# byronknoll/gmix

Measured on AMD Instinct MI355X. Metric: mixer bits/sec (synthetic 256-input mixer streams, forward+update), higher is better.
Workload: dtype f32; 1 GPU; configs[1]: synthetic 256-input 1-layer mixer (1 mixer, 2^16-row gate table), random logits, forward+update; n_inputs=256, mixers=1/0/0, streams_per_gpu=4096, total_bits=5486149632, parallelism=streams sharded over 1 GPU(s), no collective on the data path

## Files before the change

### gmix_amd/csrc/gmx_capi.cpp

```cpp
#include <hip/hip_runtime.h>
#include <math.h>
#include <stddef.h>
#include <stdio.h>
#include <stdlib.h>
#include <string.h>
#include <time.h>

#include <algorithm>
#include <atomic>
#include <map>
#include <new>
#include <string>
#include <vector>

#include "../../include/gmxmix.h"
#include "../../include/gmxmix_lstm_group.h"
#include "../../include/gmxmix_decoder.h"
#include "gmx_buildhash.h"
#include "gmx_internal.h"
#include "gmx_mailbox.h"
#include "gmx_batch_rows.h"
#include "gmx_ckpt.h"
#include "gmx_ckpt_stage.h"
#include "gmx_ind_ckpt.h"
// ... 284 lines not shown
  if (k->up) {
    const size_t bytes = (size_t)c->S * n * gmx_cols_row_bytes(c->cols, dir);
    int rc = up ? xfer_begin_upload(c->x, main, k->up, bytes, &st) : xfer_begin_download(c->x, main, k->down, bytes, &st);
    if (rc) return rc;
  }
  for (const GmxBatchCol& col : c->cols) {
    if (col.dir != dir || col.per_stream) continue;
    void *dst = up ? *col.dev : *col.host, *src = up ? *col.host : *col.dev;
    const GmxRowCopy r = gmx_row_copy(c->S, c->max_rows, n, col.row_bytes);
    if (r.height)
      HIPCHK(hipMemcpy2DAsync(dst, r.pitch, src, r.pitch, r.width, r.height, kind, st));
    else
      HIPCHK(hipMemcpyAsync(dst, src, r.bytes, kind, st));
  }
  for (const GmxBatchCol& col : c->cols) {
    if (col.dir != dir || !col.per_stream) continue;
    void *dst = up ? *col.dev : *col.host, *src = up ? *col.host : *col.dev;
    HIPCHK(hipMemcpyAsync(dst, src, gmx_col_host_bytes(col, c->S, c->max_rows), kind, st));
  }
  return up ? xfer_end_upload(c->x, main, st) : xfer_end_download(c->x, st);
}
static int batch_core_wait(GmxBatchCore* c) {
  if (!c || !c->bank) return GMX_ERR_INVALID;
  HIPCHK(hipSetDevice(c->bank->device));
  return xfer_wait(c->x);
}


static constexpr int kStageSlots = 4;
struct GmxCountList {
  uint64_t* dev[kStageSlots] = {};
  uint64_t* host[kStageSlots] = {};
  hipEvent_t done[kStageSlots] = {};
  bool busy[kStageSlots] = {};
  size_t cap = 0;
  unsigned seq = 0;
};
static void count_list_free(GmxCountList& c) {
  for (int k = 0; k < kStageSlots; ++k) {
    if (c.dev[k]) (void)hipFree(c.dev[k]);
    if (c.host[k]) (void)hipHostFree(c.host[k]);
    if (c.done[k]) (void)hipEventDestroy(c.done[k]);
  }
  c = GmxCountList();
}
static int count_list_stage(GmxCountList& c, const uint64_t* counts, int n, hipStream_t st, const uint64_t** dev_out) {
  const int k = (int)(c.seq++ % (unsigned)kStageSlots);
  if (c.busy[k]) {
    HIPCHK(hipEventSynchronize(c.done[k]));
    c.busy[k] = false;
  }
  if ((size_t)n > c.cap) {
    for (int j = 0; j < kStageSlots; ++j) {
      if (c.busy[j]) {
        HIPCHK(hipEventSynchronize(c.done[j]));
        c.busy[j] = false;
      }
      if (c.dev[j]) (void)hipFree(c.dev[j]);
      if (c.host[j]) (void)hipHostFree(c.host[j]);
      c.dev[j] = nullptr;
      c.host[j] = nullptr;
    }
    c.cap = 0;
    const size_t cap = (size_t)n + 64;
    for (int j = 0; j < kStageSlots; ++j) {
      HIPCHK(hipMalloc((void**)&c.dev[j], cap * sizeof(uint64_t)));
      HIPCHK(hipHostMalloc((void**)&c.host[j], cap * sizeof(uint64_t), hipHostMallocDefault));
      if (!c.done[j]) HIPCHK(hipEventCreateWithFlags(&c.done[j], hipEventDisableTiming));
    }
    c.cap = cap;
  }
  memcpy(c.host[k], counts, (size_t)n * sizeof(uint64_t));
  HIPCHK(hipMemcpyAsync(c.dev[k], c.host[k], (size_t)n * sizeof(uint64_t), hipMemcpyHostToDevice, st));
  *dev_out = c.dev[k];
  return GMX_OK;
}
static int count_list_used(GmxCountList& c, hipStream_t st) {
  const int k = (int)((c.seq - 1u) % (unsigned)kStageSlots);
  HIPCHK(hipEventRecord(c.done[k], st));
  c.busy[k] = true;
  return GMX_OK;
}

struct gmx_group {
  int device = 0;
  int S = 0;
  GmxTopoDev topo;
  GmxTopoDev* topo_dev = nullptr;
  uint8_t* banks = nullptr;
  float* latch_out = nullptr;
  hipStream_t stream = nullptr;
  hipEvent_t ev0 = nullptr, ev1 = nullptr;
  unsigned lds_bytes = 0;
  std::vector<uint64_t> steps;
  std::vector<uint8_t> fwd_done;
  struct DecaySlot {
    float* dev = nullptr;
    uint32_t* idx_dev = nullptr;
    float* host = nullptr;
    uint32_t* idx_host = nullptr;
    size_t cap = 0;
    size_t idx_cap = 0;
    hipEvent_t done = nullptr;
    hipEvent_t ready = nullptr;
    bool busy = false;
    uint64_t* st_dev = nullptr;
    uint64_t* st_host = nullptr;
    uint32_t* amb_dev = nullptr;
    uint32_t* amb_host = nullptr;
    float* patch_host = nullptr;
    size_t st_cap = 0;
  } decay[kStageSlots];
  GmxCountList counts;
  hipStream_t copy_stream = nullptr;
  hipStream_t up_stream = nullptr, down_stream = nullptr;
  unsigned run_seq = 0;
  hipEvent_t tm0 = nullptr, tm1 = nullptr;
  gmx_batch* one = nullptr;
  GmxBatchBank bb;
  std::vector<struct GmxSession*> sessions;
  std::vector<struct gmx_lockstep*> locksteps;
  bool banks_in_use_by_dead_kernel = false;
  bool use_sessions = true;
  bool mailbox_on_device = true;
  bool force_general = false;
  bool stock_exact = false;
  int stock_staged = -1;
  bool decay_on_host = false;
  bool stock_pairs = false;
  bool register_rows = false;
  int single_variant = 0;
  struct GmxCkptState* ckpt = nullptr;
};

struct gmx_batch : GmxBatchCore {
  gmx_group* g = nullptr;
  uint64_t& max_bits = max_rows;
  unsigned flags = 0;
  float* d_pred = nullptr;
  uint32_t* d_mask = nullptr;
  uint32_t* d_ctx = nullptr;
  uint8_t* d_bits = nullptr;
  float* d_p = nullptr;
  float* d_out = nullptr;
  float* d_last = nullptr;
  uint64_t* d_rng = nullptr;
  uint64_t* d_tcount = nullptr;
  float* d_pstate = nullptr;
  uint32_t* d_cstate = nullptr;
  float* h_pred = nullptr;
  uint32_t* h_mask = nullptr;
  uint32_t* h_ctx = nullptr;
  uint8_t* h_bits = nullptr;
  float* h_p = nullptr;
  float* h_out = nullptr;
  float* h_last = nullptr;
};

struct gmx_lockstep {
  gmx_group* g = nullptr;
  gmx_batch* b = nullptr;
  float* dec_host = nullptr;
  uint8_t* bits_host = nullptr;
  float* dec_dev = nullptr;
  uint32_t* idx_dev = nullptr;
  hipGraph_t g_predict = nullptr, g_learn = nullptr, g_step = nullptr;
  hipGraphExec_t x_predict = nullptr, x_learn = nullptr, x_step = nullptr;
  bool predicted = false;
  bool persistent = false, ps_running = false, ps_dead = false, ps_counted = false;
  hipStream_t ps_stream = nullptr;
  GmxLsDoor* door = nullptr;
  uint32_t* done = nullptr;
  uint32_t* blk_seen = nullptr;
// ... 125 lines not shown
      x.rs_off = x.w_off + (uint64_t)at * 4u;
      x.rs_pitch = x.stride * 4u;
    } else {
      x.rs_off = off;
      x.rs_pitch = 8u;
      off += (uint64_t)x.table_size * 8u;
      off = round_up64(off, 128);
    }
  }
  o->scal_off = off;
  off += (uint64_t)o->m * 24u;
  o->bank_bytes = round_up64(off, 256);
  uint32_t l = 0;
  o->lds_in0 = l;
  o->in0_sz = round_up((uint32_t)o->n_pad + (uint32_t)o->l0 + 4u, 4);
  l += 2 * o->in0_sz;
  o->lds_o1 = l;
  l += round_up((uint32_t)(o->l1 ? o->l1 : 1), 4);
  o->lds_skip = l;
  l += GMX_MAX_SKIP;
  o->lds_misc = l;
  l += 256;
  for (int grp = 0; grp < 2; ++grp) {
    const int lo = grp == 0 ? 0 : o->l0, hi = grp == 0 ? o->l0 : o->m;
    if (lo >= hi) continue;
    uint32_t dmax = 0;
    for (int j = lo; j < hi; ++j) dmax = std::max(dmax, o->mx[j].stride);
    const uint32_t D = dmax + 4;
    const uint32_t S = round_up((uint32_t)(hi - lo) * D, 64);
    for (int j = lo; j < hi; ++j) {
      o->mx[j].lds_off = l + (uint32_t)(j - lo) * D;
      o->mx[j].pitch = S;
    }
    l += 2 * S;
  }
  o->lds_total = l;
  if ((uint64_t)o->lds_total * 4u > 160u * 1024u) return GMX_ERR_INVALID;
  return GMX_OK;
}

static void batch_free(gmx_batch* b);
static int batch_alloc(gmx_batch** out, gmx_group* g, int S, uint64_t max_bits, unsigned flags);
static int batch_note_device_use(gmx_batch* b);

extern "C" int gmx_group_create(gmx_group** out, const gmx_topology* topo, int n_streams, int device) {
  if (!out || n_streams < 1) return GMX_ERR_INVALID;
  *out = nullptr;
  GmxTopoDev td;
  int rc = build_topology(topo, &td);
  if (rc) return rc;
  int ndev = 0;
  if (hipGetDeviceCount(&ndev) != hipSuccess || ndev <= 0) {
    (void)hipGetLastError();
    return GMX_ERR_NO_DEVICE;
  }
  if (device < 0 || device >= ndev) return GMX_ERR_INVALID;
  HIPCHK(hipSetDevice(device));
  gmx_group* g = new (std::nothrow) gmx_group();
  if (!g) return GMX_ERR_NOMEM;
  g->device = device;
  batch_bank_init(g->bb, g, device, &g->stream, &g->up_stream, &g->down_stream);
  g->S = n_streams;
  g->topo = td;
  g->lds_bytes = td.lds_total * 4u;
  g->steps.assign(n_streams, 0);
  g->fwd_done.assign(n_streams, 0);
#define GCHK(call)                                 \
  do {                                             \
    hipError_t e_ = (call);                        \
    if (e_ != hipSuccess) {                        \
      int r_ = hip_fail(e_, #call);                \
      gmx_group_destroy(g);                        \
      return e_ == hipErrorOutOfMemory ? GMX_ERR_NOMEM : r_; \
    }                                              \
  } while (0)
  GCHK(bank_stream_create(&g->stream, 0));
  GCHK(hipEventCreate(&g->ev0));
  GCHK(hipEventCreate(&g->ev1));
  GCHK(hipMalloc((void**)&g->topo_dev, sizeof(GmxTopoDev)));
  GCHK(hipMemcpy(g->topo_dev, &g->topo, sizeof(GmxTopoDev), hipMemcpyHostToDevice));
  GCHK(hipMalloc((void**)&g->banks, (size_t)n_streams * td.bank_bytes));
  GCHK(hipMalloc((void**)&g->latch_out, (size_t)n_streams * td.m * sizeof(float)));
  GCHK(hipMemsetAsync(g->latch_out, 0, (size_t)n_streams * td.m * sizeof(float), g->stream));
  if (g->lds_bytes > 48u * 1024u) GCHK(gmx_bank_kernel_set_lds(g->lds_bytes));
#undef GCHK
  rc = gmx_group_reset(g);
  if (rc) {
    gmx_group_destroy(g);
    return rc;
  }
  *out = g;
  return GMX_OK;
}

extern "C" void gmx_group_destroy(gmx_group* g) {
  if (!g) return;
  (void)hipSetDevice(g->device);
  sessions_free(g);
  if (g->stream) (void)hipStreamSynchronize(g->stream);
  if (g->one) {
    batch_free(g->one);
    g->one = nullptr;
  }
  for (gmx_lockstep* ls : g->locksteps) ls->g = nullptr;
  g->locksteps.clear();
  batch_bank_detach_all(g->bb);
  if (!g->banks_in_use_by_dead_kernel) {
    if (g->banks) (void)hipFree(g->banks);
    if (g->latch_out) (void)hipFree(g->latch_out);
    if (g->topo_dev) (void)hipFree(g->topo_dev);
  }
  for (auto& d : g->decay) {
    if (d.st_dev) (void)hipFree(d.st_dev);
    if (d.st_host) (void)hipHostFree(d.st_host);
    if (d.amb_dev) (void)hipFree(d.amb_dev);
    if (d.amb_host) (void)hipHostFree(d.amb_host);
    if (d.patch_host) (void)hipHostFree(d.patch_host);
    if (d.dev) (void)hipFree(d.dev);
    if (d.idx_dev) (void)hipFree(d.idx_dev);
    if (d.host) (void)hipHostFree(d.host);
    if (d.idx_host) (void)hipHostFree(d.idx_host);
    if (d.done) (void)hipEventDestroy(d.done);
    if (d.ready) (void)hipEventDestroy(d.ready);
  }
  count_list_free(g->counts);
  ckpt_free(g);
  if (g->copy_stream) (void)hipStreamDestroy(g->copy_stream);
  if (g->up_stream) {
    (void)hipStreamSynchronize(g->up_stream);
    (void)hipStreamDestroy(g->up_stream);
  }
  if (g->down_stream) {
    (void)hipStreamSynchronize(g->down_stream);
    (void)hipStreamDestroy(g->down_stream);
  }
  if (g->tm0) (void)hipEventDestroy(g->tm0);
  if (g->tm1) (void)hipEventDestroy(g->tm1);
  if (g->ev0) (void)hipEventDestroy(g->ev0);
  if (g->ev1) (void)hipEventDestroy(g->ev1);
  if (g->stream) (void)hipStreamDestroy(g->stream);
  delete g;
}

extern "C" int gmx_group_n_streams(const gmx_group* g) { return g ? g->S : GMX_ERR_INVALID; }
extern "C" int gmx_group_n_mixers(const gmx_group* g) { return g ? g->topo.m : GMX_ERR_INVALID; }
extern "C" int gmx_group_n_inputs(const gmx_group* g) { return g ? g->topo.n : GMX_ERR_INVALID; }
extern "C" uint64_t gmx_group_bank_bytes(const gmx_group* g) { return g ? g->topo.bank_bytes : 0; }

extern "C" int gmx_group_reset(gmx_group* g) {
  if (!g) return GMX_ERR_INVALID;
  HIPCHK(hipSetDevice(g->device));
  int rc = sessions_close(g, false);
  if (rc) return rc;
  HIPCHK(hipMemsetAsync(g->banks, 0, (size_t)g->S * g->topo.bank_bytes, g->stream));
  HIPCHK(gmx_launch_init_scal(g->banks, g->topo.bank_bytes, g->topo.scal_off, g->topo.m, g->S,
                              g->stream));
  HIPCHK(hipStreamSynchronize(g->stream));
  std::fill(g->steps.begin(), g->steps.end(), 0);
  std::fill(g->fwd_done.begin(), g->fwd_done.end(), 0);
  for (gmx_lockstep* ls : g->locksteps) ls->predicted = false;
  return GMX_OK;
}

extern "C" int gmx_group_sync(gmx_group* g) {
  if (!g) return GMX_ERR_INVALID;
  HIPCHK(hipSetDevice(g->device));
  int rc = sessions_close(g, true);
  if (rc) return rc;
  HIPCHK(hipStreamSynchronize(g->stream));
  return GMX_OK;
}

extern "C" int gmx_group_timer_start(gmx_group* g) {
  if (!g) return GMX_ERR_INVALID;
  HIPCHK(hipSetDevice(g->device));
  if (!g->tm0) {
    HIPCHK(hipEventCreate(&g->tm0));
    HIPCHK(hipEventCreate(&g->tm1));
  }
  HIPCHK(hipEventRecord(g->tm0, g->stream));
  return GMX_OK;
}

extern "C" int gmx_group_timer_stop(gmx_group* g, float* ms) {
  if (!g || !ms || !g->tm0) return GMX_ERR_INVALID;
  HIPCHK(hipSetDevice(g->device));
  HIPCHK(hipEventRecord(g->tm1, g->stream));
  HIPCHK(hipEventSynchronize(g->tm1));
  HIPCHK(hipEventElapsedTime(ms, g->tm0, g->tm1));
  return GMX_OK;
}

// ... 99 lines not shown
      }
      if (!e.done) {
        HIPCHK(hipEventCreateWithFlags(&e.done, hipEventDisableTiming));
        HIPCHK(hipEventCreateWithFlags(&e.ready, hipEventDisableTiming));
      }
    }
  }
  if (!g->copy_stream) HIPCHK(sibling_stream_create(&g->copy_stream, g->stream));
  bool on_device = false;
  if (learn && uniq.size() > 1 && uniq.size() * T >= kDecayDeviceMin && uniq.size() * T < (1ull << 32) &&
      !g->decay_on_host) {
    const int rcd = decay_table_on_device(g, d, uniq, T);
    if (rcd != GMX_OK && rcd != GMX_ERR_STATE) return rcd;
    on_device = rcd == GMX_OK;
  }
  if (!on_device) {
    for (auto& kv : uniq) {
      float* tab = d.host + (size_t)kv.second * T;
      if (learn)
        for (uint64_t t = 0; t < T; ++t) tab[t] = decay_base(kv.first + t);
      else
        for (uint64_t t = 0; t < T; ++t) tab[t] = 0.f;
    }
    HIPCHK(hipMemcpyAsync(d.dev, d.host, uniq.size() * T * sizeof(float), hipMemcpyHostToDevice, g->copy_stream));
  }
  memcpy(d.idx_host, idx.data(), ns * sizeof(uint32_t));
  HIPCHK(hipMemcpyAsync(d.idx_dev, d.idx_host, ns * sizeof(uint32_t), hipMemcpyHostToDevice, g->copy_stream));
  HIPCHK(hipEventRecord(d.ready, g->copy_stream));
  HIPCHK(hipStreamWaitEvent(g->stream, d.ready, 0));
  return GMX_OK;
}

static bool topo_register_rows_eligible(const GmxTopoDev& t) {
  return t.has_final && t.l0 >= 1 && t.l0 <= 24 && t.l1 >= 1 && t.l1 <= 8 && t.m == t.l0 + t.l1 + 1 &&
         t.n_skip == 1 && gmx_pair_kernel_half(t.n) != 0;
}

enum GmxKernelKind : int { GMX_K_SINGLE, GMX_K_WIDE, GMX_K_STOCK, GMX_K_BANK, GMX_K_PAIR };
static GmxKernelKind kernel_for(const gmx_group* g, unsigned mode) {
  if (g->register_rows && (mode & GMX_MODE_PREDICT) && !(mode & GMX_MODE_LATCH) && !g->force_general &&
      topo_register_rows_eligible(g->topo))
    return GMX_K_PAIR;
  const bool single = g->topo.m == 1 && g->topo.n <= 256 && (mode & GMX_MODE_PREDICT) &&
                      !(mode & GMX_MODE_LATCH) && !g->force_general;
  const bool stock = g->topo.n == 90 && g->topo.l0 == 24 && g->topo.l1 == 8 && g->topo.n_skip == 1 &&
                     g->topo.has_final && g->topo.mx[23].stride == 128 && !g->force_general;
  const bool wide = g->topo.l0 == 24 && g->topo.l1 == 8 && g->topo.n_skip == 1 && g->topo.has_final &&
                    ((g->topo.n == 256 && g->topo.mx[23].stride == 288) ||
                     (g->topo.n == 90 && g->topo.mx[23].stride == 128 && g->stock_pairs && !g->stock_exact)) &&
                    (mode & GMX_MODE_PREDICT) && !(mode & GMX_MODE_LATCH) && !g->force_general;
  return single ? GMX_K_SINGLE : wide ? GMX_K_WIDE : stock ? GMX_K_STOCK : GMX_K_BANK;
}

static int launch_run(gmx_group* g, gmx_batch* b, int s0, int rec0, int ns, uint64_t T,
                      unsigned mode, float* kernel_ms, const uint64_t* n_list = nullptr) {
  if (T == 0) return GMX_OK;
  for (gmx_lockstep* ls : g->locksteps) ls->predicted = false;
  gmx_group::DecaySlot* dec = nullptr;
  int rc = prepare_decay(g, s0, ns, T, (mode & GMX_MODE_LEARN) ? 1 : 0, &dec);
  if (rc) return rc;
  GmxRunArgs a;
  memset(&a, 0, sizeof a);
  a.banks = g->banks;
  a.pred = b->d_pred;
  a.mask = (b->flags & GMX_BATCH_MASK) ? b->d_mask : nullptr;
  a.ctx = b->d_ctx;
  a.bits = b->d_bits;
  a.decay = dec->dev;
  a.decay_idx = dec->idx_dev;
  a.p_out = b->d_p;
  a.out_all = (b->flags & GMX_BATCH_OUTPUTS) ? b->d_out : nullptr;
  a.out_last = (b->flags & GMX_BATCH_LAST_OUTPUTS) ? b->d_last : nullptr;
  a.latch_out = g->latch_out;
  a.rec_stride = b->max_bits;
  a.T = T;
  if (n_list) {
    int rcl = count_list_stage(g->counts, n_list, ns, g->stream, &a.T_list);
    if (rcl) return rcl;
  }
  a.mode = mode | (g->stock_exact ? GMX_MODE_EXACT : 0u);
  a.stream_base = s0;
  a.rec_base = rec0;
  a.n_streams = ns;
  {
    int rcx = xfer_before_run(b->x, g->stream);
    if (rcx) return rcx;
  }
  if (kernel_ms) HIPCHK(hipEventRecord(g->ev0, g->stream));
  const GmxKernelKind kind = kernel_for(g, mode);
  const bool single = kind == GMX_K_SINGLE, wide = kind == GMX_K_WIDE, stock = kind == GMX_K_STOCK;
  if (a.out_last && (single || wide)) return GMX_ERR_INVALID;
  if (kind == GMX_K_PAIR)
    HIPCHK(gmx_launch_pair_kernel(g->topo_dev, &a, ns, a.mask != nullptr, g->topo.n, g->topo.l0, g->topo.l1, g->stream));
  else if (single)
    HIPCHK(gmx_launch_single_kernel(g->topo_dev, &a, g->topo.n, g->single_variant, g->stream));
  else if (wide)
    HIPCHK(gmx_launch_wide_kernel(g->topo_dev, &a, ns, a.mask != nullptr, g->topo.n, g->stream));
  else if (stock)
    HIPCHK(gmx_launch_stock_kernel(g->topo_dev, &a, ns, GMX_STK_LDS_BYTES(g->topo.lds_misc),
                                   a.mask != nullptr, g->stock_staged, topo_tables_pow2(g->topo), g->stream));
  else
    HIPCHK(gmx_launch_bank_kernel(g->topo_dev, &a, ns, g->lds_bytes, a.mask != nullptr, g->topo.l0,
                                  g->topo.l1, g->topo.n_skip, g->topo.has_final,
                                  g->topo.mx[g->topo.l0 - 1].stride, g->stream));
  HIPCHK(hipEventRecord(dec->done, g->stream));
  dec->busy = true;
  if (n_list) {
    int rcl = count_list_used(g->counts, g->stream);
    if (rcl) return rcl;
  }
  {
    int rcn = batch_note_device_use(b);
    if (rcn) return rcn;
  }
  if (kernel_ms) {
    HIPCHK(hipEventRecord(g->ev1, g->stream));
    HIPCHK(hipEventSynchronize(g->ev1));
    HIPCHK(hipEventElapsedTime(kernel_ms, g->ev0, g->ev1));
  }
  if (mode & GMX_MODE_LEARN)
    for (int i = 0; i < ns; ++i) g->steps[s0 + i] += n_list ? n_list[i] : T;
  return GMX_OK;
}

static void batch_free(gmx_batch* b) {
  if (!b) return;
  batch_core_free(*b);
  delete b;
}

static int batch_alloc(gmx_batch** out, gmx_group* g, int S, uint64_t max_bits, unsigned flags) {
  if (!out || !g || max_bits == 0) return GMX_ERR_INVALID;
  *out = nullptr;
  gmx_batch* b = new (std::nothrow) gmx_batch();
  if (!b) return GMX_ERR_NOMEM;
  b->back = (void**)&b->g;
  b->flags = flags;
  gmx_mixer_batch_cols(b->cols, b, g->topo.n_pad, g->topo.m, g->topo.mask_words, flags);
  int rc = batch_core_alloc(*b, &g->bb, S, max_bits, false);
  if (rc) {
    batch_free(b);
    return rc;
  }
  *out = b;
  return GMX_OK;
}

extern "C" int gmx_batch_create(gmx_batch** out, gmx_group* g, uint64_t max_bits, unsigned flags) {
  if (!g) return GMX_ERR_INVALID;
  if (flags & GMX_BATCH_LAST_OUTPUTS) {
    const GmxKernelKind kind = kernel_for(g, GMX_MODE_PREDICT | GMX_MODE_LEARN);
    if ((kind == GMX_K_SINGLE || kind == GMX_K_WIDE) && !topo_register_rows_eligible(g->topo)) return GMX_ERR_INVALID;
  }
  int rc = batch_alloc(out, g, g->S, max_bits, flags);
  if (rc) return rc;
  return xfer_streams_ready(g->stream, &g->up_stream, &g->down_stream);
}

extern "C" void gmx_batch_destroy(gmx_batch* b) { batch_free(b); }
extern "C" int gmx_batch_n_pad(const gmx_batch* b) { return (b && b->g) ? b->g->topo.n_pad : GMX_ERR_INVALID; }
extern "C" int gmx_batch_mask_words(const gmx_batch* b) { return (b && b->g) ? b->g->topo.mask_words : GMX_ERR_INVALID; }
extern "C" uint64_t gmx_batch_max_bits(const gmx_batch* b) { return b ? b->max_bits : 0; }

extern "C" float* gmx_batch_predictions(gmx_batch* b) { return b ? (float*)batch_core_host(*b, &b->h_pred) : nullptr; }
extern "C" uint32_t* gmx_batch_active_mask(gmx_batch* b) {
  return b ? (uint32_t*)batch_core_host(*b, &b->h_mask) : nullptr;
// ... 260 lines not shown
      memcpy(rs, p + 4, 8);
      if (*rs == 0) return GMX_ERR_FORMAT;
      memcpy(w + (size_t)r * x.stride, p + 12, 4 * (size_t)input_size);
      p += 12 + 4 * (size_t)input_size;
    }
  }
  if (p != end) return GMX_ERR_FORMAT;
  HIPCHK(hipSetDevice(g->device));
  int rc = sessions_close(g, true);
  if (rc) return rc;
  if (stream < (int)g->sessions.size() && g->sessions[stream]) g->sessions[stream]->fwd_live = false;
  HIPCHK(hipStreamSynchronize(g->stream));
  HIPCHK(hipMemcpy(g->banks + (size_t)stream * t.bank_bytes, img.data(), img.size(),
                   hipMemcpyHostToDevice));
  g->steps[stream] = sc[0];
  g->fwd_done[stream] = 0;
  for (gmx_lockstep* ls : g->locksteps) ls->predicted = false;
  return GMX_OK;
}

extern "C" int gmx_bank_copy(gmx_group* dst, int dst_stream, gmx_group* src, int src_stream) {
  if (!dst || !src || dst_stream < 0 || dst_stream >= dst->S || src_stream < 0 || src_stream >= src->S)
    return GMX_ERR_INVALID;
  const GmxTopoDev &a = dst->topo, &b = src->topo;
  if (a.m != b.m || a.n != b.n || a.n_skip != b.n_skip || a.bank_bytes != b.bank_bytes)
    return GMX_ERR_INVALID;
  for (int j = 0; j < a.m; ++j)
    if (a.mx[j].table_size != b.mx[j].table_size || a.mx[j].weight_size != b.mx[j].weight_size ||
        a.mx[j].layer != b.mx[j].layer)
      return GMX_ERR_INVALID;
  HIPCHK(hipSetDevice(src->device));
  int rc = sessions_close(src, true);
  if (rc) return rc;
  HIPCHK(hipStreamSynchronize(src->stream));
  HIPCHK(hipSetDevice(dst->device));
  rc = sessions_close(dst, true);
  if (rc) return rc;
  if (dst_stream < (int)dst->sessions.size() && dst->sessions[dst_stream])
    dst->sessions[dst_stream]->fwd_live = false;
  HIPCHK(hipStreamSynchronize(dst->stream));
  HIPCHK(hipMemcpy(dst->banks + (size_t)dst_stream * a.bank_bytes,
                   src->banks + (size_t)src_stream * b.bank_bytes, a.bank_bytes,
                   hipMemcpyDeviceToDevice));
  dst->steps[dst_stream] = src->steps[src_stream];
  dst->fwd_done[dst_stream] = 0;
  for (gmx_lockstep* ls : dst->locksteps) ls->predicted = false;
  return GMX_OK;
}

#include "gmx_ckpt.inc"

extern "C" int gmx_bank_memory_usage(gmx_group* g, int stream, int mixer, uint64_t* bytes) {
  if (!g || stream < 0 || stream >= g->S || mixer < 0 || mixer >= g->topo.m || !bytes)
    return GMX_ERR_INVALID;
  HIPCHK(hipSetDevice(g->device));
  int rc = sessions_close(g, true);
  if (rc) return rc;
  HIPCHK(hipStreamSynchronize(g->stream));
  uint64_t sc[3];
  HIPCHK(hipMemcpy(sc, g->banks + (size_t)stream * g->topo.bank_bytes + g->topo.scal_off + 24u * mixer,
                   24, hipMemcpyDeviceToHost));
  const GmxMixerDev& x = g->topo.mx[mixer];
  *bytes = 29 + sc[2] * (uint64_t)(x.weight_size * 4 + 12) + 8ull * x.table_size;
  return GMX_OK;
}


#include "gmx_indirect.inc"
#include "gmx_ind_ckpt.inc"
#include "gmx_lstm.inc"
#include "gmx_lstm_ckpt.inc"
#include "gmx_match.inc"
#include "gmx_match_ckpt.inc"
#include "gmx_ctx.inc"
#include "gmx_ctx_ckpt.inc"
#include "gmx_chainstep.inc"
#include "gmx_coder.inc"

extern "C" int gmx_debug_single_variant(gmx_group* g, int lanes_per_stream) {
  if (!g || (lanes_per_stream != 0 && lanes_per_stream != 16 && lanes_per_stream != 32 &&
             lanes_per_stream != 64 && lanes_per_stream != 165 && lanes_per_stream != 325))
    return GMX_ERR_INVALID;
  g->single_variant = lanes_per_stream;
  return GMX_OK;
}

extern "C" int gmx_debug_stock_pairs(gmx_group* g, int on) {
  if (!g) return GMX_ERR_INVALID;
  g->stock_pairs = on != 0;
  return GMX_OK;
}

extern "C" int gmx_debug_decay_on_host(gmx_group* g, int on) {
  if (!g) return GMX_ERR_INVALID;
  g->decay_on_host = on != 0;
  return GMX_OK;
}

extern "C" int gmx_debug_decay_table(gmx_group* g, const uint64_t* steps0, int U, uint64_t T, float* out,
                                     uint32_t* n_unsettled) {
  if (!g || !steps0 || U < 1 || T < 1 || !out) return GMX_ERR_INVALID;
  HIPCHK(hipSetDevice(g->device));
  if (!g->copy_stream) HIPCHK(sibling_stream_create(&g->copy_stream, g->stream));
  gmx_group::DecaySlot tmp;
  std::map<uint64_t, uint32_t> uniq;
  std::vector<uint32_t> row(U);
  for (int u = 0; u < U; ++u) {
    auto it = uniq.find(steps0[u]);
    if (it == uniq.end()) it = uniq.emplace(steps0[u], (uint32_t)uniq.size()).first;
    row[u] = it->second;
  }
  HIPCHK(hipMalloc((void**)&tmp.dev, uniq.size() * T * sizeof(float)));
  int rc = decay_table_on_device(g, tmp, uniq, T);
  if (rc == GMX_OK) {
    if (n_unsettled) *n_unsettled = tmp.amb_host[0];
    std::vector<float> h(uniq.size() * T);
    hipError_t e = hipMemcpyAsync(h.data(), tmp.dev, h.size() * sizeof(float), hipMemcpyDeviceToHost, g->copy_stream);
    if (e == hipSuccess) e = hipStreamSynchronize(g->copy_stream);
    if (e != hipSuccess) rc = hip_fail(e, "gmx_debug_decay_table copy");
    else
      for (int u = 0; u < U; ++u) memcpy(out + (size_t)u * T, h.data() + (size_t)row[u] * T, T * sizeof(float));
  }
  void* dv[] = {tmp.dev, tmp.st_dev, tmp.amb_dev};
  for (void* p : dv)
    if (p) (void)hipFree(p);
  void* hv[] = {tmp.st_host, tmp.amb_host, tmp.patch_host};
  for (void* p : hv)
    if (p) (void)hipHostFree(p);
  return rc;
}

extern "C" int gmx_topology_register_rows_eligible(const gmx_topology* topo) {
  GmxTopoDev td;
  if (build_topology(topo, &td) != GMX_OK) return GMX_ERR_INVALID;
  return topo_register_rows_eligible(td) ? 1 : 0;
}

extern "C" int gmx_group_set_register_rows(gmx_group* g, int on) {
  if (!g || !topo_register_rows_eligible(g->topo)) return GMX_ERR_INVALID;
  g->register_rows = on != 0;
  return GMX_OK;
}

extern "C" int gmx_debug_force_general(gmx_group* g, int on) {
  if (!g) return GMX_ERR_INVALID;
  g->force_general = on != 0;
  return GMX_OK;
}

extern "C" int gmx_debug_kernel_kind(gmx_group* g, unsigned mode) {
  if (!g) return GMX_ERR_INVALID;
  const GmxKernelKind kind = kernel_for(g, mode);
  if (kind != GMX_K_BANK) return (int)kind;
  const GmxTopoDev& t = g->topo;
  return (int)kind + 4 * gmx_bank_kernel_build(t.l0, t.l1, t.n_skip, t.has_final, t.mx[t.l0 - 1].stride);
}

extern "C" int gmx_debug_stock_staged(gmx_group* g, int mode) {
  if (!g || mode < -1 || mode > 1) return GMX_ERR_INVALID;
  g->stock_staged = mode;
  return GMX_OK;
}

extern "C" int gmx_debug_stock_exact(gmx_group* g, int on) {
  if (!g) return GMX_ERR_INVALID;
  int rc = sessions_close(g, true);
// ... 511 lines not shown
```

### gmix_amd/csrc/gmx_internal.h

```cpp
#ifndef GMX_INTERNAL_H_
#define GMX_INTERNAL_H_

#include <stdint.h>

#define GMX_MAX_MIXERS 64
#define GMX_MAX_SKIP 8
#define GMX_MAX_INPUTS 2048

#define GMX_MODE_PREDICT 1u
#define GMX_MODE_LEARN 2u
#define GMX_MODE_LATCH 4u
#define GMX_MODE_EXACT 8u

struct GmxMixerDev {
  uint32_t table_size;
  uint32_t weight_size;
  uint32_t stride;
  uint32_t lds_off;
  uint32_t pitch;
  int32_t layer;
  int32_t out_index;
  float lr;
  uint64_t w_off;
  uint64_t rs_off;
  uint32_t rs_pitch;
  uint32_t rs_folded;
};

#define GMX_RS_PTR(bank, mx, row) \
  ((uint64_t*)((uint8_t*)(bank) + (mx).rs_off + (uint64_t)(row) * (mx).rs_pitch))

struct GmxTopoDev {
  int32_t n, n_pad, n_skip, m, l0, l1, has_final, mask_words;
  int32_t skip_idx[GMX_MAX_SKIP];
  uint32_t lds_in0;
  uint32_t in0_sz;
  uint32_t lds_o1;
  uint32_t lds_skip;
  uint32_t lds_misc;
  uint32_t lds_total;
  uint64_t scal_off;
  uint64_t bank_bytes;
  GmxMixerDev mx[GMX_MAX_MIXERS];
};

struct GmxRunArgs {
  uint8_t* banks;
  const float* pred;
  const uint32_t* mask;
  const uint32_t* ctx;
  const uint8_t* bits;
  const float* decay;
  const uint32_t* decay_idx;
  float* p_out;
  float* out_all;
  float* out_last;
  float* latch_out;
  uint64_t rec_stride;
  uint64_t T;
  const uint64_t* T_list;
  uint32_t mode;
  int32_t stream_base;
  int32_t rec_base;
  int32_t n_streams;
};

#define GMX_STK_LDS_BYTES(lds_misc) (((lds_misc) + 256u) * 4u + 2u * 33u * 528u)

#define GMX_MB_FORWARD 1u
#define GMX_MB_LEARN0 2u
#define GMX_MB_LEARN1 3u
#define GMX_MB_STOP 4u
#define GMX_MB_LEARN0_FWD 5u
#define GMX_MB_LEARN1_FWD 6u
#define GMX_MB_STOP_KEEP 7u
#define GMX_MB_CMD_MASK 7u
#define GMX_MB_SLOT_SHIFT 3
#define GMX_MB_SEQ_SHIFT 4
#define GMX_MB_RUNNING 0u
#define GMX_MB_EXIT_IDLE 1u
#define GMX_MB_EXIT_STOP 2u
struct GmxMbPayload {
  uint32_t dec_bits;
  uint32_t pad0[3];
  uint32_t mask[4];
  uint32_t ctx[36];
  uint32_t pad1[4];
  float pred[96];
};
struct GmxMbCmd {
  uint32_t cmd_seq;
  uint32_t pad0[15];
  GmxMbPayload slot[2];
};
struct GmxMbReply {
  uint32_t done_seq;
  uint32_t state;
  float p;
  uint32_t pad[13];
  float outs[48];
};

struct GmxLsDoor {
  uint32_t cmd_seq;
  uint32_t pad[15];
};
struct GmxLsArgs {
  uint8_t* banks;
  GmxLsDoor* door;
  uint32_t* done;
  const float* pred;
  const uint32_t* mask;
  const uint32_t* ctx;
  const uint8_t* bits;
  const float* dec;
  float* p;
  float* outs;
  uint32_t* blk_seen;
  uint32_t* blk_replay;
  uint32_t* relay;
  float* live;
  uint64_t idle_ticks;
  int32_t n_streams, exact;
};
#define GMX_LS_LIVE_FLOATS 160

struct GmxStkStepArgs {
  uint8_t* banks;
  const uint8_t* what;
  const uint8_t* bits;
  const float* dec;
  const float* pred_old;
  const uint32_t* mask_old;
  const uint32_t* ctx_old;
  const float* pred_new;
  const uint32_t* mask_new;
  const uint32_t* ctx_new;
  float* p_out;
  float* out_all;
  float* latch;
  const uint32_t* seq;
  uint32_t* stamp;
  int32_t n_streams, exact;
};

#define GMX_STEP_UP_MAX 12
struct GmxStepUpload {
// ... 183 lines not shown
```

### gmix_amd/csrc/gmx_single.hip

```cpp
#include <hip/hip_runtime.h>
#include <stdint.h>

#include "gmx_internal.h"
#include "gmx_math.h"

typedef float gmx_f4 __attribute__((ext_vector_type(4)));

template <int OFF>
__device__ __forceinline__ void gmx_ld16(gmx_f4& d, const float* p) {
  asm volatile("global_load_dwordx4 %0, %1, off offset:%2 nt" : "=v"(d) : "v"(p), "n"(OFF) : "memory");
}
__device__ __forceinline__ void gmx_ld8(uint64_t& d, const uint64_t* p) {
  asm volatile("global_load_dwordx2 %0, %1, off" : "=v"(d) : "v"(p) : "memory");
}
__device__ __forceinline__ void gmx_ld4(uint32_t& d, const void* p) {
  asm volatile("global_load_dword %0, %1, off" : "=v"(d) : "v"(p) : "memory");
}
__device__ __forceinline__ void gmx_ld1(uint32_t& d, const uint8_t* p) {
  asm volatile("global_load_ubyte %0, %1, off" : "=v"(d) : "v"(p) : "memory");
}
template <int OFF>
__device__ __forceinline__ void gmx_st16(float* p, const gmx_f4& v) {
  asm volatile("global_store_dwordx4 %0, %1, off offset:%2 nt" : : "v"(p), "v"(v), "n"(OFF) : "memory");
}
__device__ __forceinline__ void gmx_st8(uint64_t* p, uint64_t v) {
  asm volatile("global_store_dwordx2 %0, %1, off" : : "v"(p), "v"(v) : "memory");
}
__device__ __forceinline__ void gmx_st4(float* p, float v) {
  asm volatile("global_store_dword %0, %1, off" : : "v"(p), "v"(v) : "memory");
}

template <int K>
struct GmxSlot {
  gmx_f4 w[K];
  gmx_f4 x[K];
  uint32_t mk[K];
  uint64_t rs;
  uint32_t row;
  uint32_t bit;
  uint32_t dec;
};

template <int N>
__device__ __forceinline__ void gmx_wait_slot(GmxSlot<1>& a) {
  asm volatile("s_waitcnt vmcnt(%c5)"
               : "+v"(a.w[0]), "+v"(a.x[0]), "+v"(a.rs), "+v"(a.bit), "+v"(a.dec)
               : "n"(N));
}
template <int N>
__device__ __forceinline__ void gmx_wait_slot(GmxSlot<2>& a) {
  asm volatile("s_waitcnt vmcnt(%c7)"
               : "+v"(a.w[0]), "+v"(a.w[1]), "+v"(a.x[0]), "+v"(a.x[1]), "+v"(a.rs), "+v"(a.bit),
                 "+v"(a.dec)
               : "n"(N));
}
template <int N>
__device__ __forceinline__ void gmx_wait_slot(GmxSlot<4>& a) {
  asm volatile("s_waitcnt vmcnt(%c11)"
               : "+v"(a.w[0]), "+v"(a.w[1]), "+v"(a.w[2]), "+v"(a.w[3]), "+v"(a.x[0]), "+v"(a.x[1]),
                 "+v"(a.x[2]), "+v"(a.x[3]), "+v"(a.rs), "+v"(a.bit), "+v"(a.dec)
               : "n"(N));
}
template <int K>
__device__ __forceinline__ void gmx_pin_mask(GmxSlot<K>& a) {
  if (K == 1) asm volatile("" : "+v"(a.mk[0]));
  if (K == 2) asm volatile("" : "+v"(a.mk[0]), "+v"(a.mk[1 % K]));
  if (K == 4) asm volatile("" : "+v"(a.mk[0]), "+v"(a.mk[1 % K]), "+v"(a.mk[2 % K]), "+v"(a.mk[3 % K]));
}
__device__ __forceinline__ void gmx_pin(uint64_t& rs, uint32_t& bit, uint32_t& dec, uint32_t& cq) {
  asm volatile("" : "+v"(rs), "+v"(bit), "+v"(dec), "+v"(cq));
}

template <int LPS>
__device__ __forceinline__ float gmx_handoff(float acc, int i, bool first_pass, int lane) {
  const int a = __float_as_int(acc);
  if (LPS == 64)
    return __int_as_float(__builtin_amdgcn_update_dpp(0, a, 0x13C, 0xf, 0xf, false));
  if (LPS == 16)
    return __int_as_float(__builtin_amdgcn_update_dpp(0, a, 0x121, 0xf, 0xf, false));
  if (i == 16)
    return __int_as_float(__builtin_amdgcn_update_dpp(a, a, 0x142, 0xa, 0xf, false));
  if (i == 0 && !first_pass)
    return __shfl(acc, (lane & 32) | 31);
  return __int_as_float(__builtin_amdgcn_update_dpp(0, a, 0x121, 0xf, 0xf, false));
}

template <int K, int LPS>
__device__ __forceinline__ float gmx_chain_piece(const GmxSlot<K>& c, int q, float acc, int lane) {
  const float px = c.x[q].x * c.w[q].x, py = c.x[q].y * c.w[q].y;
  const float pz = c.x[q].z * c.w[q].z, pw = c.x[q].w * c.w[q].w;
#pragma unroll
  for (int i = 0; i < LPS; ++i) {
    acc = gmx_handoff<LPS>(acc, i, q == 0, lane) + px;
    acc = acc + py;
    acc = acc + pz;
    acc = acc + pw;
  }
  return acc;
}
template <int K, int LPS>
__device__ __forceinline__ float gmx_chain(const GmxSlot<K>& c, int lane) {
  float acc = 0.f;
#pragma unroll
  for (int q = 0; q < K; ++q) acc = gmx_chain_piece<K, LPS>(c, q, acc, lane);
  return acc;
}

template <int LPS, int K, int NSLOT, bool FULL, bool WANT_OUT, bool LEARN, bool HAS_MASK>
__global__ void __launch_bounds__(64)
gmx_single_kernel(const GmxTopoDev* __restrict__ tp, const GmxRunArgs a) {
  constexpr int G = 64 / LPS;
  constexpr int CH = 4 * LPS;
  constexpr int VM_PER_BIT = 1 + (WANT_OUT ? 1 : 0) + (LEARN ? K + 1 : 0) + 2 * K + 3 + (HAS_MASK ? K : 0) + 1;
  constexpr int VM_WAIT = 1 + (NSLOT - 2) * VM_PER_BIT;
  static_assert(VM_WAIT <= 63, "vmcnt is a 6-bit counter");
  static_assert(CH * 4 * (K - 1) < 4096, "immediate offset of global_load is 12 bits");
  const int lane = threadIdx.x;
  const int g = lane / LPS, l = lane % LPS;
  const int li = (int)blockIdx.x * G + g;
  __shared__ uint64_t s_tab[32];
  if (lane < 32) s_tab[lane] = gmx_exp2f_tab[lane];
  if (li >= a.n_streams) return;
  const int rec = a.rec_base + li;
  const int s = a.stream_base + li;
  const uint64_t T = a.T;
  if (T == 0) return;

  const int N = tp->n, NPAD = tp->n_pad;
  const uint32_t stride = FULL ? (uint32_t)(CH * K) : tp->mx[0].stride;
  const uint32_t table = tp->mx[0].table_size;
  const float lr = tp->mx[0].lr;
  uint8_t* const bank = a.banks + (uint64_t)s * tp->bank_bytes;
  float* const wtab = (float*)(bank + tp->mx[0].w_off);
  uint64_t* const rstab = (uint64_t*)(bank + tp->mx[0].rs_off);
  uint64_t* const scal = (uint64_t*)(bank + tp->scal_off);

  const uint64_t RS = a.rec_stride;
  const uint32_t xstride = FULL ? (uint32_t)(CH * K) : (uint32_t)NPAD;
  const float* const pred_s = a.pred + (uint64_t)rec * RS * xstride;
  const uint32_t* const ctx_s = a.ctx + (uint64_t)rec * RS;
  const uint8_t* const bits_s = a.bits + (uint64_t)rec * RS;
  const float* const dec_s = a.decay + (uint64_t)a.decay_idx[li] * T;
  const int MW = tp->mask_words;
  const uint32_t* const mask_s = HAS_MASK ? a.mask + (uint64_t)rec * RS * MW : nullptr;
  float* const p_s = a.p_out + (uint64_t)rec * RS;
  float* const oa_s = WANT_OUT ? a.out_all + (uint64_t)rec * RS : nullptr;

  uint64_t steps = scal[0], max_steps = scal[1], seen_cnt = scal[2];

  GmxSlot<K> sl[NSLOT];
  uint32_t ctxq[NSLOT];

  auto issue = [&](GmxSlot<K>& d, uint32_t ctx, uint64_t tb) {
    const uint64_t tt = tb < T ? tb : T - 1;
    d.row = ctx % table;
    const float* wr = wtab + (uint64_t)d.row * stride + 4 * l;
    const float* xr = pred_s + tt * (uint64_t)xstride + 4 * l;
    if (FULL) {
      gmx_ld16<0>(d.w[0], wr);
      if (K > 1) gmx_ld16<CH * 4>(d.w[1 % K], wr);
      if (K > 2) gmx_ld16<CH * 8>(d.w[2 % K], wr);
      if (K > 3) gmx_ld16<CH * 12>(d.w[3 % K], wr);
      gmx_ld16<0>(d.x[0], xr);
      if (K > 1) gmx_ld16<CH * 4>(d.x[1 % K], xr);
      if (K > 2) gmx_ld16<CH * 8>(d.x[2 % K], xr);
      if (K > 3) gmx_ld16<CH * 12>(d.x[3 % K], xr);
    } else {
#pragma unroll
      for (int k = 0; k < K; ++k) {
        const int e = CH * k + 4 * l;
        gmx_ld16<0>(d.w[k], (uint32_t)e < stride ? wr + CH * k : wr - 4 * l);
      }
#pragma unroll
      for (int k = 0; k < K; ++k) {
        const int e = CH * k + 4 * l;
        gmx_ld16<0>(d.x[k], e < NPAD ? xr + CH * k : xr - 4 * l);
      }
    }
    if (HAS_MASK) {
#pragma unroll
      for (int k = 0; k < K; ++k) {
        const int e = CH * k + 4 * l;
        gmx_ld4(d.mk[k], mask_s + tt * (uint64_t)MW + (e < NPAD ? (e >> 5) : 0));
      }
    }
    gmx_ld8(d.rs, rstab + d.row);
    gmx_ld1(d.bit, bits_s + tt);
    gmx_ld4(d.dec, dec_s + tt);
  };
  auto mask_inputs = [&](GmxSlot<K>& d) {
    if (!HAS_MASK) return;
#pragma unroll
    for (int k = 0; k < K; ++k) {
      const uint32_t b = d.mk[k] >> ((uint32_t)(CH * k + 4 * l) & 31u);
      d.x[k].x = (b & 1u) ? d.x[k].x : 0.f;
      d.x[k].y = (b & 2u) ? d.x[k].y : 0.f;
      d.x[k].z = (b & 4u) ? d.x[k].z : 0.f;
      d.x[k].w = (b & 8u) ? d.x[k].w : 0.f;
    }
  };
  auto trim = [&](GmxSlot<K>& d) {
    if (FULL) return;
#pragma unroll
    for (int k = 0; k < K; ++k) {
      const int e = CH * k + 4 * l;
      const bool wok = (uint32_t)e < stride;
      d.w[k].x = wok ? d.w[k].x : 0.f;
      d.w[k].y = wok ? d.w[k].y : 0.f;
      d.w[k].z = wok ? d.w[k].z : 0.f;
      d.w[k].w = wok ? d.w[k].w : 0.f;
      d.x[k].x = (e + 0 < N) ? d.x[k].x : 0.f;
      d.x[k].y = (e + 1 < N) ? d.x[k].y : 0.f;
      d.x[k].z = (e + 2 < N) ? d.x[k].z : 0.f;
      d.x[k].w = (e + 3 < N) ? d.x[k].w : 0.f;
    }
  };

#pragma unroll
  for (int k = 0; k < NSLOT; ++k) {
    const uint64_t tb = (uint64_t)k < T ? (uint64_t)k : T - 1;
    ctxq[k] = ctx_s[tb];
  }
#pragma unroll
  for (int k = 0; k < NSLOT; ++k) {
    issue(sl[k], ctxq[k], (uint64_t)k);
    const uint64_t tb = (uint64_t)(k + NSLOT) < T ? (uint64_t)(k + NSLOT) : T - 1;
    gmx_ld4(ctxq[k], ctx_s + tb);
  }
#pragma unroll
  for (int k = 0; k < NSLOT; ++k) {
    gmx_wait_slot<0>(sl[k]);
    if (HAS_MASK) gmx_pin_mask(sl[k]);
    gmx_pin(sl[k].rs, sl[k].bit, sl[k].dec, ctxq[k]);
  }
  trim(sl[0]);
  mask_inputs(sl[0]);
  float acc_cur = gmx_chain<K, LPS>(sl[0], lane);

  for (uint64_t t0 = 0; t0 < T; t0 += NSLOT) {
#pragma unroll
    for (int k = 0; k < NSLOT; ++k) {
      const uint64_t t = t0 + k;
      if (t >= T) break;
      GmxSlot<K>& c = sl[k];
      GmxSlot<K>& nx = sl[(k + 1) % NSLOT];
      gmx_wait_slot<VM_WAIT>(nx);
      if (HAS_MASK) gmx_pin_mask(nx);
      gmx_pin(c.rs, c.bit, c.dec, ctxq[k]);
      trim(nx);
      mask_inputs(nx);
      float acc_nxt = gmx_chain_piece<K, LPS>(nx, 0, 0.f, lane);
      float out = __shfl(acc_cur, lane | (LPS - 1));
      const bool seen = c.rs != 0;
      out = seen ? out : 0.f;
      const float pl = gmx_logistic_tab(out, s_tab);
      const float prob = gmx_clamp_prob(pl);
      gmx_st4(p_s + t, prob);
      if (WANT_OUT) gmx_st4(oa_s + t, out);
      if (K > 1) acc_nxt = gmx_chain_piece<K, LPS>(nx, 1 % K, acc_nxt, lane);
      if (!LEARN) {
        if (K > 2) acc_nxt = gmx_chain_piece<K, LPS>(nx, 2 % K, acc_nxt, lane);
        if (K > 3) acc_nxt = gmx_chain_piece<K, LPS>(nx, 3 % K, acc_nxt, lane);
      } else {
        const double dd = (double)__uint_as_float(c.dec) * (1.5 - ((double)c.rs) / (double)max_steps);
        const float decay = (float)dd;
        const float upd = decay * lr * (pl - (float)c.bit);
        const uint64_t rs_new = c.rs + 1;
        ++steps;
        max_steps = rs_new > max_steps ? rs_new : max_steps;
        seen_cnt += (c.rs == 0) ? 1u : 0u;
        const float sc = ((rs_new & 1023u) == 0) ? (1.0f - 3.0e-6f) : 1.0f;
        if (K > 2) acc_nxt = gmx_chain_piece<K, LPS>(nx, 2 % K, acc_nxt, lane);
#pragma unroll
        for (int q = 0; q < K; ++q) {
          c.w[q].x = (c.w[q].x - upd * c.x[q].x) * sc;
          c.w[q].y = (c.w[q].y - upd * c.x[q].y) * sc;
          c.w[q].z = (c.w[q].z - upd * c.x[q].z) * sc;
          c.w[q].w = (c.w[q].w - upd * c.x[q].w) * sc;
        }
        float* wr = wtab + (uint64_t)c.row * stride + 4 * l;
        if (FULL) {
          gmx_st16<0>(wr, c.w[0]);
          if (K > 1) gmx_st16<CH * 4>(wr, c.w[1 % K]);
          if (K > 2) gmx_st16<CH * 8>(wr, c.w[2 % K]);
          if (K > 3) gmx_st16<CH * 12>(wr, c.w[3 % K]);
        } else {
#pragma unroll
          for (int q = 0; q < K; ++q)
            if ((uint32_t)(CH * q + 4 * l) < stride) gmx_st16<0>(wr + CH * q, c.w[q]);
        }
        gmx_st8(rstab + c.row, rs_new);
        if (K > 3) acc_nxt = gmx_chain_piece<K, LPS>(nx, 3 % K, acc_nxt, lane);
        bool hit[NSLOT];
        bool any_hit = false;
#pragma unroll
        for (int j = 1; j < NSLOT; ++j) {
          hit[j] = sl[(k + j) % NSLOT].row == c.row && (t + j) < T;
          any_hit |= hit[j];
        }
        if (__any(any_hit)) {
#pragma unroll
          for (int j = 2; j < NSLOT; ++j) gmx_wait_slot<0>(sl[(k + j) % NSLOT]);
#pragma unroll
          for (int j = 1; j < NSLOT; ++j) {
            GmxSlot<K>& o = sl[(k + j) % NSLOT];
            if (hit[j]) {
#pragma unroll
              for (int q = 0; q < K; ++q) o.w[q] = c.w[q];
              o.rs = rs_new;
            }
          }
          if (__any(hit[1])) acc_nxt = gmx_chain<K, LPS>(nx, lane);
        }
      }
      issue(c, ctxq[k], t + NSLOT);
      {
        const uint64_t tn = t + 2 * NSLOT;
        gmx_ld4(ctxq[k], ctx_s + (tn < T ? tn : T - 1));
      }
      acc_cur = acc_nxt;
    }
  }
  asm volatile("s_waitcnt vmcnt(0)" ::: "memory");
  if (LEARN) {
    scal[0] = steps;
    scal[1] = max_steps;
    scal[2] = seen_cnt;
  }
}

template <int LPS, int K, int NSLOT, bool FULL, bool HAS_MASK>
static hipError_t launch_kfm(const GmxTopoDev* tp_dev, const GmxRunArgs& a, hipStream_t stream) {
  constexpr int G = 64 / LPS;
  const dim3 grid((a.n_streams + G - 1) / G), block(64);
  const bool learn = (a.mode & GMX_MODE_LEARN) != 0;
  if (a.out_all) {
    if (learn)
      hipLaunchKernelGGL((gmx_single_kernel<LPS, K, NSLOT, FULL, true, true, HAS_MASK>), grid, block, 0, stream, tp_dev, a);
    else
      hipLaunchKernelGGL((gmx_single_kernel<LPS, K, NSLOT, FULL, true, false, HAS_MASK>), grid, block, 0, stream, tp_dev, a);
  } else {
    if (learn)
      hipLaunchKernelGGL((gmx_single_kernel<LPS, K, NSLOT, FULL, false, true, HAS_MASK>), grid, block, 0, stream, tp_dev, a);
    else
      hipLaunchKernelGGL((gmx_single_kernel<LPS, K, NSLOT, FULL, false, false, HAS_MASK>), grid, block, 0, stream, tp_dev, a);
  }
  return hipGetLastError();
}
template <int LPS, int K, int NSLOT, bool FULL>
static hipError_t launch_kf(const GmxTopoDev* tp_dev, const GmxRunArgs& a, hipStream_t stream) {
  constexpr int VM_M = 1 + 1 + (K + 1) + 2 * K + 3 + K + 1;
  constexpr int NS_M = (1 + (NSLOT - 2) * VM_M <= 63) ? NSLOT : NSLOT - 1;
  return a.mask ? launch_kfm<LPS, K, NS_M, FULL, true>(tp_dev, a, stream)
                : launch_kfm<LPS, K, NSLOT, FULL, false>(tp_dev, a, stream);
}

template <int LPS, int K, int NSLOT>
static hipError_t launch_k(const GmxTopoDev* tp_dev, const GmxRunArgs& a, bool full,
                           hipStream_t stream) {
  return full ? launch_kf<LPS, K, NSLOT, true>(tp_dev, a, stream)
              : launch_kf<LPS, K, NSLOT, false>(tp_dev, a, stream);
}

extern "C" hipError_t gmx_launch_single_kernel(const GmxTopoDev* tp_dev, const GmxRunArgs* args,
                                               int n_inputs, int variant, hipStream_t stream) {
  (void)hipGetLastError();
  const GmxRunArgs& a = *args;
  if (n_inputs <= 64) return launch_k<16, 1, 4>(tp_dev, a, n_inputs == 64, stream);
  if (n_inputs <= 128) {
    if (variant == 16) return launch_k<16, 2, 4>(tp_dev, a, n_inputs == 128, stream);
    return launch_k<32, 1, 6>(tp_dev, a, n_inputs == 128, stream);
  }
  const bool full = n_inputs == 256;
  if (variant == 165) return launch_k<16, 4, 5>(tp_dev, a, full, stream);
  if (variant == 325) return launch_k<32, 2, 5>(tp_dev, a, full, stream);
  if (variant == 64) return launch_k<64, 1, 6>(tp_dev, a, full, stream);
  if (variant == 32) return launch_k<32, 2, 4>(tp_dev, a, full, stream);
  return launch_k<16, 4, 4>(tp_dev, a, full, stream);
}
```

Before: 1.836 billion bits/s.

## Prefetch row-step counters one slot-round ahead and skip weight loads for fresh rows

The single-stream kernel now loads the per-row step counter (rstab) one pipeline round earlier than the weights, keeping a second queue of rows and counters. It then uses that counter when issuing the weight load: rows never touched (rs==0) read from a shared zeroed device row instead of the table, which cuts scattered global traffic for cold rows. Forwarding for in-flight rows is extended to the new counter queue, the vmcnt accounting is adjusted, and ctx prefetch moves one round further ahead. This adds register pressure and extra waits on hit paths; the non-full 165 variant drops to 4 slots. A debug query for the zero row is added.

```diff
diff --git a/gmix_amd/csrc/gmx_capi.cpp b/gmix_amd/csrc/gmx_capi.cpp
--- a/gmix_amd/csrc/gmx_capi.cpp
+++ b/gmix_amd/csrc/gmx_capi.cpp
@@ -390,6 +390,8 @@
   return GMX_OK;
 }
 
+static const size_t kZeroRowBytes = 4096;
+
 struct gmx_group {
   int device = 0;
   int S = 0;
@@ -397,6 +399,8 @@
   GmxTopoDev* topo_dev = nullptr;
   uint8_t* banks = nullptr;
   float* latch_out = nullptr;
+  uint8_t* zero_row_mem = nullptr;
+  const float* zero_row = nullptr;
   hipStream_t stream = nullptr;
   hipEvent_t ev0 = nullptr, ev1 = nullptr;
   unsigned lds_bytes = 0;
@@ -688,6 +692,9 @@
   GCHK(hipMalloc((void**)&g->banks, (size_t)n_streams * td.bank_bytes));
   GCHK(hipMalloc((void**)&g->latch_out, (size_t)n_streams * td.m * sizeof(float)));
   GCHK(hipMemsetAsync(g->latch_out, 0, (size_t)n_streams * td.m * sizeof(float), g->stream));
+  GCHK(hipMalloc((void**)&g->zero_row_mem, kZeroRowBytes + 1024));
+  GCHK(hipMemsetAsync(g->zero_row_mem, 0, kZeroRowBytes + 1024, g->stream));
+  g->zero_row = (const float*)(((uintptr_t)g->zero_row_mem + 1023u) & ~(uintptr_t)1023u);
   if (g->lds_bytes > 48u * 1024u) GCHK(gmx_bank_kernel_set_lds(g->lds_bytes));
 #undef GCHK
   rc = gmx_group_reset(g);
@@ -714,6 +721,7 @@
   if (!g->banks_in_use_by_dead_kernel) {
     if (g->banks) (void)hipFree(g->banks);
     if (g->latch_out) (void)hipFree(g->latch_out);
+    if (g->zero_row_mem) (void)hipFree(g->zero_row_mem);
     if (g->topo_dev) (void)hipFree(g->topo_dev);
   }
   for (auto& d : g->decay) {
@@ -979,6 +987,7 @@
   a.stream_base = s0;
   a.rec_base = rec0;
   a.n_streams = ns;
+  a.zero_row = g->zero_row;
   {
     int rcx = xfer_before_run(b->x, g->stream);
     if (rcx) return rcx;
@@ -1405,6 +1414,18 @@
              lanes_per_stream != 64 && lanes_per_stream != 165 && lanes_per_stream != 325))
     return GMX_ERR_INVALID;
   g->single_variant = lanes_per_stream;
+  return GMX_OK;
+}
+
+extern "C" int gmx_debug_zero_row_nonzero(gmx_group* g, uint32_t* count) {
+  if (!g || !count || !g->zero_row) return GMX_ERR_INVALID;
+  HIPCHK(hipSetDevice(g->device));
+  HIPCHK(hipStreamSynchronize(g->stream));
+  std::vector<uint8_t> h(kZeroRowBytes);
+  HIPCHK(hipMemcpy(h.data(), g->zero_row, kZeroRowBytes, hipMemcpyDeviceToHost));
+  uint32_t n = 0;
+  for (uint8_t v : h) n += v != 0;
+  *count = n;
   return GMX_OK;
 }
 
diff --git a/gmix_amd/csrc/gmx_internal.h b/gmix_amd/csrc/gmx_internal.h
--- a/gmix_amd/csrc/gmx_internal.h
+++ b/gmix_amd/csrc/gmx_internal.h
@@ -63,6 +63,7 @@
   int32_t stream_base;
   int32_t rec_base;
   int32_t n_streams;
+  const float* zero_row;
 };
 
 #define GMX_STK_LDS_BYTES(lds_misc) (((lds_misc) + 256u) * 4u + 2u * 33u * 528u)
diff --git a/gmix_amd/csrc/gmx_single.hip b/gmix_amd/csrc/gmx_single.hip
--- a/gmix_amd/csrc/gmx_single.hip
+++ b/gmix_amd/csrc/gmx_single.hip
@@ -12,6 +12,14 @@
 }
 __device__ __forceinline__ void gmx_ld8(uint64_t& d, const uint64_t* p) {
   asm volatile("global_load_dwordx2 %0, %1, off" : "=v"(d) : "v"(p) : "memory");
+}
+__device__ __forceinline__ void gmx_ld8_inplace(uint64_t& d, const uint64_t* p) {
+  asm volatile("global_load_dwordx2 %0, %1, off" : "+v"(d) : "v"(p) : "memory");
+}
+__device__ __forceinline__ uint64_t gmx_take8(const uint64_t& s) {
+  uint64_t d;
+  asm volatile("v_mov_b64 %0, %1" : "=&v"(d) : "v"(s));
+  return d;
 }
 __device__ __forceinline__ void gmx_ld4(uint32_t& d, const void* p) {
   asm volatile("global_load_dword %0, %1, off" : "=v"(d) : "v"(p) : "memory");
@@ -69,6 +77,10 @@
 }
 __device__ __forceinline__ void gmx_pin(uint64_t& rs, uint32_t& bit, uint32_t& dec, uint32_t& cq) {
   asm volatile("" : "+v"(rs), "+v"(bit), "+v"(dec), "+v"(cq));
+}
+
+__device__ __forceinline__ void gmx_wait_rs(uint64_t& rs) {
+  asm volatile("s_waitcnt vmcnt(0)" : "+v"(rs));
 }
 
 template <int LPS>
@@ -111,7 +123,7 @@
 gmx_single_kernel(const GmxTopoDev* __restrict__ tp, const GmxRunArgs a) {
   constexpr int G = 64 / LPS;
   constexpr int CH = 4 * LPS;
-  constexpr int VM_PER_BIT = 1 + (WANT_OUT ? 1 : 0) + (LEARN ? K + 1 : 0) + 2 * K + 3 + (HAS_MASK ? K : 0) + 1;
+  constexpr int VM_PER_BIT = 1 + (WANT_OUT ? 1 : 0) + (LEARN ? K + 1 : 0) + 1 + 2 * K + 2 + (HAS_MASK ? K : 0) + 1;
   constexpr int VM_WAIT = 1 + (NSLOT - 2) * VM_PER_BIT;
   static_assert(VM_WAIT <= 63, "vmcnt is a 6-bit counter");
   static_assert(CH * 4 * (K - 1) < 4096, "immediate offset of global_load is 12 bits");
@@ -148,13 +160,18 @@
 
   uint64_t steps = scal[0], max_steps = scal[1], seen_cnt = scal[2];
 
+  const float* const zrow = a.zero_row + 4 * l;
+
   GmxSlot<K> sl[NSLOT];
+  uint64_t rsq[NSLOT];
+  uint32_t rowq[NSLOT];
   uint32_t ctxq[NSLOT];
 
-  auto issue = [&](GmxSlot<K>& d, uint32_t ctx, uint64_t tb) {
+  auto issue = [&](GmxSlot<K>& d, uint32_t row, uint64_t rs, uint64_t tb) {
     const uint64_t tt = tb < T ? tb : T - 1;
-    d.row = ctx % table;
-    const float* wr = wtab + (uint64_t)d.row * stride + 4 * l;
+    d.row = row;
+    d.rs = rs;
+    const float* wr = rs != 0 ? wtab + (uint64_t)row * stride + 4 * l : zrow;
     const float* xr = pred_s + tt * (uint64_t)xstride + 4 * l;
     if (FULL) {
       gmx_ld16<0>(d.w[0], wr);
@@ -184,7 +201,6 @@
         gmx_ld4(d.mk[k], mask_s + tt * (uint64_t)MW + (e < NPAD ? (e >> 5) : 0));
       }
     }
-    gmx_ld8(d.rs, rstab + d.row);
     gmx_ld1(d.bit, bits_s + tt);
     gmx_ld4(d.dec, dec_s + tt);
   };
@@ -216,26 +232,35 @@
     }
   };
 
+  uint32_t row0[NSLOT];
+  uint64_t rs0[NSLOT];
 #pragma unroll
   for (int k = 0; k < NSLOT; ++k) {
-    const uint64_t tb = (uint64_t)k < T ? (uint64_t)k : T - 1;
-    ctxq[k] = ctx_s[tb];
-  }
+    const uint64_t ta = (uint64_t)k < T ? (uint64_t)k : T - 1;
+    const uint64_t tb = (uint64_t)(k + NSLOT) < T ? (uint64_t)(k + NSLOT) : T - 1;
+    row0[k] = ctx_s[ta] % table;
+    rowq[k] = ctx_s[tb] % table;
+  }
+#pragma unroll
+  for (int k = 0; k < NSLOT; ++k) rs0[k] = rstab[row0[k]];
 #pragma unroll
   for (int k = 0; k < NSLOT; ++k) {
-    issue(sl[k], ctxq[k], (uint64_t)k);
-    const uint64_t tb = (uint64_t)(k + NSLOT) < T ? (uint64_t)(k + NSLOT) : T - 1;
+    rsq[k] = 0;
+    gmx_ld8_inplace(rsq[k], rstab + rowq[k]);
+    issue(sl[k], row0[k], rs0[k], (uint64_t)k);
+    const uint64_t tb = (uint64_t)(k + 2 * NSLOT) < T ? (uint64_t)(k + 2 * NSLOT) : T - 1;
     gmx_ld4(ctxq[k], ctx_s + tb);
   }
 #pragma unroll
   for (int k = 0; k < NSLOT; ++k) {
     gmx_wait_slot<0>(sl[k]);
     if (HAS_MASK) gmx_pin_mask(sl[k]);
-    gmx_pin(sl[k].rs, sl[k].bit, sl[k].dec, ctxq[k]);
+    gmx_pin(rsq[k], sl[k].bit, sl[k].dec, ctxq[k]);
   }
   trim(sl[0]);
   mask_inputs(sl[0]);
   float acc_cur = gmx_chain<K, LPS>(sl[0], lane);
+  asm volatile("" : "+v"(steps), "+v"(max_steps), "+v"(seen_cnt));
 
   for (uint64_t t0 = 0; t0 < T; t0 += NSLOT) {
 #pragma unroll
@@ -246,7 +271,7 @@
       GmxSlot<K>& nx = sl[(k + 1) % NSLOT];
       gmx_wait_slot<VM_WAIT>(nx);
       if (HAS_MASK) gmx_pin_mask(nx);
-      gmx_pin(c.rs, c.bit, c.dec, ctxq[k]);
+      gmx_pin(rsq[k], c.bit, c.dec, ctxq[k]);
       trim(nx);
       mask_inputs(nx);
       float acc_nxt = gmx_chain_piece<K, LPS>(nx, 0, 0.f, lane);
@@ -291,16 +316,23 @@
         }
         gmx_st8(rstab + c.row, rs_new);
         if (K > 3) acc_nxt = gmx_chain_piece<K, LPS>(nx, 3 % K, acc_nxt, lane);
-        bool hit[NSLOT];
+        bool hit[NSLOT], hitq[NSLOT];
         bool any_hit = false;
 #pragma unroll
         for (int j = 1; j < NSLOT; ++j) {
           hit[j] = sl[(k + j) % NSLOT].row == c.row && (t + j) < T;
           any_hit |= hit[j];
         }
+#pragma unroll
+        for (int j = 0; j < NSLOT; ++j) {
+          hitq[j] = rowq[(k + j) % NSLOT] == c.row && (t + NSLOT + j) < T;
+          any_hit |= hitq[j];
+        }
         if (__any(any_hit)) {
 #pragma unroll
           for (int j = 2; j < NSLOT; ++j) gmx_wait_slot<0>(sl[(k + j) % NSLOT]);
+#pragma unroll
+          for (int j = 0; j < NSLOT; ++j) gmx_wait_rs(rsq[j]);
 #pragma unroll
           for (int j = 1; j < NSLOT; ++j) {
             GmxSlot<K>& o = sl[(k + j) % NSLOT];
@@ -310,12 +342,19 @@
               o.rs = rs_new;
             }
           }
+#pragma unroll
+          for (int j = 0; j < NSLOT; ++j)
+            if (hitq[j]) rsq[(k + j) % NSLOT] = rs_new;
           if (__any(hit[1])) acc_nxt = gmx_chain<K, LPS>(nx, lane);
         }
       }
-      issue(c, ctxq[k], t + NSLOT);
       {
-        const uint64_t tn = t + 2 * NSLOT;
+        const uint32_t row_n = rowq[k];
+        const uint64_t rs_n = gmx_take8(rsq[k]);
+        rowq[k] = ctxq[k] % table;
+        gmx_ld8_inplace(rsq[k], rstab + rowq[k]);
+        issue(c, row_n, rs_n, t + NSLOT);
+        const uint64_t tn = t + 3 * NSLOT;
         gmx_ld4(ctxq[k], ctx_s + (tn < T ? tn : T - 1));
       }
       acc_cur = acc_nxt;
@@ -372,7 +411,8 @@
     return launch_k<32, 1, 6>(tp_dev, a, n_inputs == 128, stream);
   }
   const bool full = n_inputs == 256;
-  if (variant == 165) return launch_k<16, 4, 5>(tp_dev, a, full, stream);
+  if (variant == 165)
+    return full ? launch_kf<16, 4, 5, true>(tp_dev, a, stream) : launch_kf<16, 4, 4, false>(tp_dev, a, stream);
   if (variant == 325) return launch_k<32, 2, 5>(tp_dev, a, full, stream);
   if (variant == 64) return launch_k<64, 1, 6>(tp_dev, a, full, stream);
   if (variant == 32) return launch_k<32, 2, 4>(tp_dev, a, full, stream);
```

After: 1.835 billion bits/s, median of 2. About the same (-0.0%).
